# PacificBiosciences/ccs

Measured on AMD Instinct MI355X. Metric: ZMWs/sec (HiFi reads/sec), 10-pass x 10 kb synthetic, higher is better.
Workload: dtype f32

## Files before the change

ccs_amd/csrc/ccsx_api.cpp:

```cpp
#include <hip/hip_runtime.h>

#include <algorithm>
#include <cmath>
#include <cstdio>
#include <cstdlib>
#include <cstring>
#include <initializer_list>
#include <mutex>
#include <string>
#include <vector>

#include "ccsx.h"
#include "ccsx_internal.h"
#include "ccsx_kernels.h"

#define HIPTRY(expr)                                                                                           \
    do {                                                                                                       \
        hipError_t e_ = (expr);                                                                                \
        if (e_ != hipSuccess) {                                                                                \
            ccsx_set_error(std::string(#expr) + ": " + hipGetErrorString(e_));                                 \
            return -2;                                                                                         \
        }                                                                                                      \
    } while (0)

// ... 124 lines not shown
    int device = 0;
    hipStream_t s_in = nullptr, s_draft = nullptr, s_comp = nullptr, s_out = nullptr;
    hipStream_t s_aux = nullptr;
    hipEvent_t ev_epoch = nullptr, ev_epoch_nx = nullptr;
    float age_ms = 0.0f;
    double epoch_ms = 0.0;
    bool poisoned = false;
    ccsx_model model;
    ccsx_opts opts;
    DevBuf d_model, d_poa, d_align;
    DevBuf d_hd_lf;
    Slot slot[CCSX_SLOTS];
    int last = 0;
    int64_t next_ticket = 0;
    int handles_on_device = 1;
};

static void finish_outputs(const Slot &S, ccsx_results *res, ccsx_drafts *d)
{
    const int n = S.P.n_zmw;
    if (res && res->seq_off) std::memcpy(res->seq_off, S.seq_off.p, (size_t)(n + 1) * 8);
    if (d) {
        std::memcpy(d->seq_off, S.seq_off.p, (size_t)(n + 1) * 8);
        if (d->win_off) for (int z = 0; z <= n; ++z) d->win_off[z] = S.wb_off[z];
        for (int z = 0; z < n; ++z) d->backbone[z] &= 255;
    }
}

static int slot_timings(ccsx_handle h, Slot &S, ccsx_timings *t)
{
// ... 87 lines not shown
    else HIPTRY(hipStreamCreateWithFlags(&h->s_comp, hipStreamNonBlocking));
    if (h->opts.serial_stages) h->s_draft = h->s_comp;
    else if (pe) HIPTRY(hipStreamCreateWithPriority(&h->s_draft, hipStreamNonBlocking, p_draft));
    else HIPTRY(hipStreamCreateWithFlags(&h->s_draft, hipStreamNonBlocking));
    HIPTRY(hipStreamCreateWithFlags(&h->s_out, hipStreamNonBlocking));
    { const char *e = getenv("CCSX_POA_SPLIT"); if (((!h->opts.serial_stages && pe) || (e && !strcmp(e, "2"))) && !(e && !strcmp(e, "0"))) { if (pe) HIPTRY(hipStreamCreateWithPriority(&h->s_aux, hipStreamNonBlocking, p_draft)); else HIPTRY(hipStreamCreateWithFlags(&h->s_aux, hipStreamNonBlocking)); } }
    HIPTRY(hipEventCreate(&h->ev_epoch));
    HIPTRY(hipEventCreate(&h->ev_epoch_nx));
    HIPTRY(hipEventRecord(h->ev_epoch, h->s_draft));
    for (auto &s : h->slot) {
        for (auto &ev : s.ev) HIPTRY(hipEventCreate(&ev));
        for (auto &ev : s.ev_aux) HIPTRY(hipEventCreateWithFlags(&ev, hipEventDisableTiming));
        HIPTRY(hipEventCreateWithFlags(&s.ev_up, hipEventDisableTiming));
        HIPTRY(hipEventCreateWithFlags(&s.ev_done, hipEventDisableTiming));
    }
    if (h->d_model.reserve(sizeof(ccsx_model))) return -2;
    HIPTRY(hipMemcpy(h->d_model.p, &h->model, sizeof(ccsx_model), hipMemcpyHostToDevice));
    return 0;
}

int ccsx_create(int device_ordinal, const ccsx_model *model, const ccsx_opts *opts, ccsx_handle *out)
{
    if (!model || !opts || !out) { ccsx_set_error("ccsx_create: null argument"); return -1; }
    int n = 0;
    hipError_t e = hipGetDeviceCount(&n);
    if (e != hipSuccess || n <= 0) { ccsx_set_error("ccsx_create: no HIP device available (this library has no CPU fallback)"); return -2; }
    if (device_ordinal < 0 || device_ordinal >= n) { ccsx_set_error("ccsx_create: bad device ordinal"); return -1; }
    HIPTRY(hipSetDevice(device_ordinal));
    hipDeviceProp_t prop;
    HIPTRY(hipGetDeviceProperties(&prop, device_ordinal));
// ... 275 lines not shown
        if ((P.sdust_words = sdust_mask_words(h, S)) < 0) return -1;
    }
    if ((rc = upload_inputs(S, b, kin, st, P)) || (rc = reserve_state(S, (size_t)n, (size_t)R, kin, pile, W.tandem, P))) return rc;
    if ((rc = grow_scratch(h, n, R, T, P))) return rc;
    P.n_zmw = n; P.n_reads = R; P.maxL_max = (int32_t)T.maxL_max; P.vcap_max = (int32_t)T.vcap_max; P.need_max = T.need_max; P.max_reads = T.nr_max;
    P.n_quads = T.n_quads; P.total_wslots = T.total_wslots;
    P.opts = h->opts;
    P.perr_floor = ccsx_perr_floor(h->opts.max_qv);
    P.model = (const ccsx_model *)h->d_model.p;
    if (ccsx_polish_lds(T.nr_max, &P.pw_obs_bytes, &P.pw_gb_floats)) { ccsx_set_error("ccsx_upload: cannot size the polish kernel's LDS"); return -2; }
    S.P = P;
    S.staged = true; S.ran = false; S.tm_ok = false;
    return 0;
}

static int launch(ccsx_handle h, Slot &S)
{
    (void)hipGetLastError();
    KParams &P = S.P;
    if ((size_t)P.poa_slots * P.poa_slot_bytes > h->d_poa.cap) P.poa_slots = (int)slots_that_fit(h->d_poa.cap, P.poa_slot_bytes, 1);
    const size_t words = h->d_align.cap / 4;
    if ((size_t)P.align_slots * P.align_slot_i32 + align16_words(P.align16_regions, P.align16_slots, P.align16_slot_i32) > words) {
        if ((size_t)P.align_slots * P.align_slot_i32 > words / 2) P.align_slots = (int)slots_that_fit(words / 2, P.align_slot_i32, 1);
        const size_t used = (size_t)P.align_slots * P.align_slot_i32, left = words > used ? words - used : 0;
        P.align16_slots = (int)slots_that_fit(left, (size_t)P.align16_regions * P.align16_slot_i32, 1);
    }
    bind_scratch(h, P);
    if (!h->d_poa.p || !h->d_align.p) { ccsx_set_error("kernel launch refused: the POA / alignment scratch is not allocated (an earlier allocation failed)"); return -2; }
    const char *failed = ccsx_launch_all(S.P, {h->s_draft, h->s_comp, h->s_aux, S.ev, h->s_aux ? S.ev_aux : nullptr}, S.mode);
    if (failed) { ccsx_set_error(std::string("kernel launch failed: ") + failed); return -2; }
    S.ran = true;
    return 0;
}

static int check_results(const Slot &S, const ccsx_results *res, bool have_kin)
{
    const int n = S.P.n_zmw;
    if (!res || res->n_zmw != n || res->seq_capacity < S.seq_off[n]) { ccsx_set_error("ccsx_download: result buffers too small"); return -1; }
    if (!have_kin && (res->fi || res->fp || res->ri || res->rp)) {
        ccsx_set_error("ccsx_download: kinetics buffers given but the handle was created without opts.hifi_kinetics");
        return -1;
    }
    return 0;
}
// ... 859 lines not shown
```

ccs_amd/csrc/ccsx_host.cpp:

```cpp
#include "ccsx.h"
#include "ccsx_internal.h"

int ccsx_kernel_is_experiment();
const char *ccsx_kernel_build_flags();

#include <atomic>
#include <algorithm>
#include <cmath>
#include <thread>
#include <cstdlib>
#include <cstring>
#include <cctype>
#include <cstdio>
#include <sched.h>
#include <string>
#include <vector>

static thread_local std::string g_last_error;
void ccsx_set_error(const std::string &s) { g_last_error = s; }

extern "C" {

int ccsx_abi_version(void) { return CCSX_ABI_VERSION; }
int ccsx_spec_version(void) { return ccsx_kernel_is_experiment() ? -CCSX_SPEC_VERSION : CCSX_SPEC_VERSION; }
const char *ccsx_build_flags(void) { return ccsx_kernel_build_flags(); }
const char *ccsx_last_error(void) { return g_last_error.c_str(); }
const char *ccsx_runtime_switches(void)
{
    static const char *names[] = {"CCSX_STAGE_PRIO", "CCSX_POA_SPLIT", "CCSX_SERIAL_STAGES", "CCSX_A16_ONE_REGION", "CCSX_ALIGN16_MAX_SLOTS", "CCSX_TB_ASIDE",
                                  "CCSX_POLISH_MAX_BLOCKS", "CCSX_EPOCH_REBASE_MS", "CCSX_TRACE", "CCSX_NUMA", "CCSX_INFLATE_PRIO"};
    static thread_local std::string out;
    out.clear();
    for (const char *n : names)
        if (const char *v = std::getenv(n)) { if (!out.empty()) out += ' '; out += n; out += '='; out += v; }
    return out.c_str();
}

void ccsx_model_default(ccsx_model *m)
{
    std::memset(m, 0, sizeof(*m));
    std::strncpy(m->name, "SYN-1", sizeof(m->name) - 1);
    m->snr_lo = 4.0f;
    m->snr_hi = 20.0f;
    static const float pw_match[3] = {0.30f, 0.30f, 0.40f};
    static const float pw_extra[3] = {0.60f, 0.25f, 0.15f};
// ... 248 lines not shown
```

ccs_amd/csrc/ccsx_kernels.h:

```cpp
#pragma once
#include <hip/hip_runtime.h>
#include <stdint.h>
#include <math.h>

#include "ccsx.h"

#define CCSX_POA_BYTES_PER_VERTEX 238

static inline float ccsx_perr_floor(int max_qv) { return max_qv == 50 ? 1e-5f : (float)pow(10.0, -(double)max_qv / 10.0); }

#define CCSX_TB_WORDS_PER_BLOCK 18
static inline __host__ __device__ int ccsx_tb_blocks(int Ld) { return (Ld + 15) >> 4; }
static inline __host__ __device__ int ccsx_tb_stride(int Ld) { return (ccsx_tb_blocks(Ld) * CCSX_TB_WORDS_PER_BLOCK + 3) & ~3; }

static inline __host__ __device__ int ccsx_top_passes(int top_passes) { return (top_passes <= 0 || top_passes > CCSX_MAX_PASSES) ? CCSX_MAX_PASSES : top_passes; }

struct KParams {
    int32_t n_zmw, n_reads;
    int32_t maxL_max;
    int32_t vcap_max;
    int32_t need_max;
    int32_t max_reads;
    int32_t qv_only;
    ccsx_opts opts;
// ... 133 lines not shown
    CCSX_EV_END = 5,
    CCSX_EV_POLISH_START = 6,
    CCSX_EV_COUNT
};
enum ccsx_order_event {
    CCSX_ORD_POA_FORK = 0,
    CCSX_ORD_FIRST_DP_DONE = 1,
    CCSX_ORD_POA_JOIN = 2,
    CCSX_ORD_ALIGN16_DONE_0 = 3,
    CCSX_ORD_ALIGN16_DONE_1 = 4,
    CCSX_ORD_TB_DONE_0 = 5,
    CCSX_ORD_TB_DONE_1 = 6,
    CCSX_ORD_COUNT
};

struct ccsx_launch_queues {
    hipStream_t draft, polish, aux;
    hipEvent_t *ev, *ev_aux;
};
const char *ccsx_launch_all(const KParams &P, const ccsx_launch_queues &q, int mode);
const char *ccsx_train_launch(const KParams &P, hipStream_t st, long long max_blocks);
int ccsx_kernel_is_experiment();
const char *ccsx_kernel_build_flags();
int ccsx_polish_lds(int max_reads, int *obs_bytes, int *gb_floats);
```

ccs_amd/csrc/ccsx_kernels.hip:

```cpp
#include <hip/hip_runtime.h>
#include <stdint.h>
#include <cstdio>
#include <cstdlib>

#include "ccsx.h"
#include "ccsx_kernels.h"
#include "wave_ops.h"

#define LANDED(x) asm volatile("" : "+v"(x))

#if (defined(CCSX_EXP_NO_FILL) || defined(CCSX_EXP_NO_SCORE) || defined(CCSX_EXP_ONE_ROUND) || defined(CCSX_EXP_ALL_VALID) || defined(CCSX_EXP_CHEAP_VALIDITY) || \
     defined(CCSX_EXP_NO_ROWS) || defined(CCSX_EXP_NO_SCORE_LOG) || defined(CCSX_EXP_SKIP_ROUND2_SCORE) || defined(CCSX_EXP_NO_QV_EXP) || defined(CCSX_EXP_REPEAT) || defined(CCSX_EXP_NO_BANDMASK) || \
     defined(CCSX_EXP_HOT_PROLOGUE) || defined(CCSX_EXIT_AFTER_PROLOGUE)) && !defined(CCSX_EXPERIMENT)
#error "CCSX_EXP_* / CCSX_EXIT_AFTER_PROLOGUE switches produce wrong results: build them with -DCCSX_EXPERIMENT (never ship such a library)"
#endif
#define CCSX_STR2(x) #x
#define CCSX_STR(x) CCSX_STR2(x)
int ccsx_kernel_is_experiment()
{
#ifdef CCSX_EXPERIMENT
    return 1;
#else
    return 0;
#endif
// ... 380 lines not shown
                    const int c = 8 + offs[k];
                    bool bad = false;
#pragma unroll
                    for (int p = 1; p <= 4; ++p) bad |= ((e[p - 1] >> (c - p)) & ((1u << p) - 1u)) == ((1u << p) - 1u);
                    if (!bad) nb = cur + CCSX_WIN_CORE + offs[k];
                }
            }
            ++nw;
            if (lane == 0) b[nw] = nb;
            cur = nb;
        }
    }
    return nw;
}

__global__ __launch_bounds__(64) void k_poa_init(KParams P, int z0, int pass, int b0)
{
    const int bx = (int)blockIdx.x + b0;
    const int lane = threadIdx.x;
    uint32_t *sread = dyn_lds;
    PoaSlot g = poa_slot(P, bx);
    if (z0 + bx >= P.n_zmw) return;
    const int z = rfl(P.zmw_perm[z0 + bx]);
    if (lane < ST_WORDS) g.st[lane] = 0;
    __threadfence_block();
    const int r0 = rfl(P.read_off[z]);
    int nreads = rfl(P.read_off[z + 1]) - r0;
    {
        const int top = ccsx_top_passes(P.opts.top_passes);
        if (nreads > top) nreads = top;
    }
    const int nall = nreads;
    {
        int nf = 0;
// ... 56 lines not shown
    else {
        for (int i = lane; i < I; i += LANES) {
            const int b = read_base_packed(sread, i);
            g.crec0[i] = make_int4(b | ((i > 0 ? 1 : 0) << 8) | (1 << CREC_NREADS_SHIFT), i - 1, -1, -1);
            g.needK[i] = 0;
        }
        n = I;
    }
    __threadfence_block();
    if (lane == 0) {
        g.st[ST_N] = n; g.st[ST_NADDED] = 1; g.st[ST_OK] = ok; g.st[ST_PAR] = 0; g.st[ST_KEND] = -1; g.st[ST_BS] = NEGV;
        g.st[ST_NPOA] = npoa; g.st[ST_BB] = bb; g.st[ST_NREADS] = nreads; g.st[ST_REV0] = rev0; g.st[ST_LIVE] = 1;
    }
}

__global__ __launch_bounds__(64) void k_draft_in(KParams P)
{
    const int lane = threadIdx.x, z = blockIdx.x;
    if (z >= P.n_zmw) return;
    const int r0 = rfl(P.read_off[z]);
    int nreads = rfl(P.read_off[z + 1]) - r0;
    {
        const int top = ccsx_top_passes(P.opts.top_passes);
        if (nreads > top) nreads = top;
    }
    const int nall = nreads;
    {
        int nf = 0;
        for (int b0 = 0; b0 < nall; b0 += LANES) nf += __popcll(__ballot(b0 + lane < nall && !(P.flags[r0 + (b0 + lane < nall ? b0 + lane : 0)] & 2)));
        nreads = rfl(nf);
// ... 11 lines not shown
    for (int q = lane; q < Ld; q += LANES) draft[q] = draft[q] & 3;
    __threadfence_block();
    if (stat < 0) nw = poa_windows(P, z, Ld, lane);
    for (int q = lane; q < nall; q += LANES) { P.avalid[r0 + q] = 0; P.ascore[r0 + q] = NEGV; }
    if (lane == 0) {
        P.nreads_used[z] = nall; P.nfull[z] = nreads; P.zref[z] = bb;
        P.draft_len[z] = (stat == CCSX_TOO_FEW_PASSES) ? 0 : Ld; P.nwin[z] = (stat < 0) ? nw : 0; P.zstat[z] = (stat < 0) ? CCSX_SUCCESS : stat;
    }
}

__device__ __forceinline__ void load_read_chunk_m1(uint32_t *sread, const uint8_t *bases, int L, int rev, int c0, int l16)
{
    for (int w = l16; w <= CH16 / 16 + 1; w += 16) sread[w] = pack16_bases<8>(bases, L, c0 - 1 + (w << 4), rev != 0, rev != 0);
}

__global__ __launch_bounds__(64) void k_poa_dp(KParams P, int z0, int pass, int rr, int b0)
{
    const int bx = (int)blockIdx.x + b0;
    __shared__ __attribute__((aligned(16))) int32_t sRing[4][PRING + 1][PGS];
    __shared__ __attribute__((aligned(16))) int4 sKin[4][PRING + 1];
    __shared__ __attribute__((aligned(16))) int4 sCrec[4][16];
    __shared__ uint32_t sRead[4][CH16 / 16 + 2];
    const int lane = threadIdx.x, gq = lane >> 4, l = lane & 15;
    const int zi = z0 + 4 * bx + gq;
    const bool have = zi < P.n_zmw && 4 * bx + gq < P.poa_slots;
    const PoaSlot G = poa_slot(P, have ? 4 * bx + gq : 4 * bx);
    int32_t *st = G.st;
    int32_t *Mcol = G.M;
    int4 *kinfo = G.kinfo;
    const int par_ = have ? st[ST_PAR] : 0;
    const int4 *crec = par_ ? G.crec1 : G.crec0;
    const int32_t *pxw = (const int32_t *)(par_ ? G.px1 : G.px0);
    const uint8_t *needK = G.needK;
    uint8_t *mvK = G.mvK;
    bool live = have && st[ST_LIVE] && st[ST_OK] && rr < st[ST_NPOA];
    if (!__any(live)) return;
    const int z = have ? P.zmw_perm[zi] : 0;
    const int r0 = P.read_off[z];
// ... 188 lines not shown
            if (__builtin_expect((rec.x & CREC_NEED) != 0, 0)) {
                *(int2 *)Mp = make_int2(b0, b1);
                if (l == 0) *kip = make_int4(lo, cm, br, p0);
            }
        }
    }
#undef M_NE0
#undef M_SLT
#undef M_SGT
#undef M_UGT
#undef LDS_I32
    __threadfence_block();
    if (live && l == 0) { st[ST_KEND] = kend; st[ST_BS] = bs; }
}

__global__ __launch_bounds__(64) __attribute__((amdgpu_waves_per_eu(8, 8))) void k_poa_thread(KParams P, int z0, int pass, int rr, int b0)
{
    const int bx = (int)blockIdx.x + b0;
    __shared__ __attribute__((aligned(16))) uint8_t sMv[TB_BLOCK * POA_MV_BYTES];
    const int lane = threadIdx.x;
    uint32_t *sread = dyn_lds;
    PoaSlot g = poa_slot(P, bx);
    if (z0 + bx >= P.n_zmw) return;
    if (!g.st[ST_LIVE] || !g.st[ST_OK] || rr >= g.st[ST_NPOA]) return;
    TPH_T0();
    const int z = rfl(P.zmw_perm[z0 + bx]);
    const int r0 = rfl(P.read_off[z]);
    const int bb = rfl(g.st[ST_BB]), nreads = rfl(g.st[ST_NREADS]), npoa = rfl(g.st[ST_NPOA]);
    const int r = r0 + (bb + rr < nreads ? bb + rr : bb + rr - nreads);
    const uint8_t *rb = P.bases + P.base_off[r];
    const int I = rfl((int)(P.base_off[r + 1] - P.base_off[r]));
    const int kend = rfl(g.st[ST_KEND]), bsc = rfl(g.st[ST_BS]);
    if (kend < 0 || bsc < I) return;
    const int rev = rfl(((P.flags[r] & 1) != g.st[ST_REV0]) ? 1 : 0);
    const int vcap = rfl(P.vcap[z]);
// ... 216 lines not shown
                        rec.x += 1 << 8;
                        if (P - Pp > PRING) { g.needK[Pp] = 1; if (np == 0) rec.x |= CREC_FAR0; }
                    }
                }
            }
            crec_nx[P] = rec;
            if (((rec.x >> 8) & 15) > 3 || pxdirty) px_nx[P] = pxr;
        }
    }
    __threadfence_block();
    if (lane == 0) { g.st[ST_N] = n; g.st[ST_NADDED] += 1; g.st[ST_PAR] ^= 1; }
    (void)npoa;
    TPH(13);
}

__global__ __launch_bounds__(64) __attribute__((amdgpu_waves_per_eu(8, 8))) void k_poa_finish(KParams P, int z0, int pass, int b0)
{
    const int bx = (int)blockIdx.x + b0;
    const int lane = threadIdx.x;
    PoaSlot g = poa_slot(P, bx);
    if (z0 + bx >= P.n_zmw) return;
    if (!g.st[ST_LIVE]) return;
    const int z = rfl(P.zmw_perm[z0 + bx]);
    const int ok = rfl(g.st[ST_OK]), n = rfl(g.st[ST_N]), nadded = rfl(g.st[ST_NADDED]);
    const int4 *crec = g.st[ST_PAR] ? g.crec1 : g.crec0;
    const int32_t *pxw = (const int32_t *)(g.st[ST_PAR] ? g.px1 : g.px0);
    int Ld = 0, nw = 0, stat = -1;
    if (ok && n > 0) {
        int kbest = -1, sb = NEGV, best_prev = 0;
        for (int kb = 0; kb < n; kb += LANES) {
            const int kkL = kb + lane;
            int4 cL = make_int4(0, -1, -1, -1);
            if (kkL < n) cL = crec[kkL];
            const int nblk = (n - kb) < LANES ? (n - kb) : LANES;
// ... 77 lines not shown
        __threadfence_block();
        if (len <= P.dcap[z]) {
            uint8_t *draft = P.draft + P.seq_off[z];
            for (int q = lane; q < len; q += LANES) draft[q] = tmp[len - 1 - q];
            Ld = len;
        }
        __threadfence_block();
    }
    if (Ld <= 0) stat = CCSX_DRAFT_FAILURE;
    else if (Ld < P.opts.min_length) stat = CCSX_TOO_SHORT;
    else if (Ld > P.opts.max_length) stat = CCSX_TOO_LONG;
    else {
        nw = poa_windows(P, z, Ld, lane);
    }
    if (lane == 0) { P.draft_len[z] = Ld; P.nwin[z] = (stat < 0) ? nw : 0; P.zstat[z] = (stat < 0) ? CCSX_SUCCESS : stat; }
}

__device__ __forceinline__ int need_col(const int32_t *wb, int nw, int Ld, int k)
{
    return k == 0 ? 0 : (k == 2 * nw - 1 ? Ld : wb[(k + 1) >> 1] + ((k & 1) ? -CCSX_WIN_OVERHANG : CCSX_WIN_OVERHANG));
}
struct AlignEnd { int M, O, lo; unsigned K; };
template <int REV>
__device__ __forceinline__ AlignEnd align_pass(const KParams &P, const uint32_t *sread, int I, const uint8_t *d, int Ld, const int32_t *wb, int nw,
                                               int32_t *Osave, int lane)
{
    const int nneed = 2 * nw;
    int32_t *lo_need = Osave + (size_t)P.need_max * 128;
    int32_t *cm_need = lo_need + P.need_max + 64, *br_need = cm_need + P.need_max, *eb_need = br_need + P.need_max;
    int2 *OMsave = (int2 *)Osave;
// ... 86 lines not shown
#define AVALID_TB 2
__device__ __forceinline__ int tb_blocks(int Ld) { return ccsx_tb_blocks(Ld); }
__device__ __forceinline__ int tb_stride(int Ld) { return ccsx_tb_stride(Ld); }
__device__ __forceinline__ unsigned shift_in(unsigned acc, unsigned long long m)
{
    unsigned r; unsigned long long co;
    asm("v_addc_co_u32_e64 %0, %1, %2, %2, %3" : "=v"(r), "=s"(co) : "v"(acc), "s"(m));
    return r;
}
__device__ __forceinline__ int sel_i32(unsigned long long m, int a, int b)
{
    int r;
    asm("v_cndmask_b32_e64 %0, %1, %2, %3" : "=v"(r) : "v"(b), "v"(a), "s"(m));
    return r;
}
__global__ __launch_bounds__(64) void k_align16(KParams P, int qbase, int pass, int region)
{
    const int lane = threadIdx.x, h = lane >> 4, l = lane & 15, rowb = lane & 48;
    uint32_t *sread = dyn_lds;
    uint32_t *Osave = (uint32_t *)(P.align_scratch + ((size_t)region * P.align16_slots + blockIdx.x) * P.align16_slot_i32);
    if (qbase + (int)blockIdx.x >= P.n_quads) return;
    const int qd = rfl(P.quads[qbase + blockIdx.x]);
    const int rfirst = qd >> 2, nq = (qd & 3) + 1;
    const int z = rfl(P.read_zmw[rfirst]);
    const int r0 = rfl(P.read_off[z]);
    const int zr = rfl(P.zref[z]);
    if (pass && !(zr & ZREF_PASSBIT(pass))) return;
    const bool live = h < nq;
    const int r = rfirst + (live ? h : 0);
    if (live && l == 0) { P.avalid[r] = 0; P.ascore[r] = NEGV; }
    if (P.zstat[z] != CCSX_SUCCESS) return;
    const int nused = rfl(P.nreads_used[z]);
    if (rfirst - r0 >= nused) return;
    const bool use = live && (r - r0 < nused);
    if (P.opts.disable_heuristics || (P.tflag && (rfl(P.tflag[z]) & 2))) {
        if (l == 0 && use) { const int idx = atomicAdd(&P.align_retry[0], 1); P.align_retry[16 + idx] = r; }
        return;
// ... 121 lines not shown
    const int sc = (inr && scv > -(1 << 22)) ? scv : NEGV;
    const int valid = (sc > NEGV / 2 && sc >= Ld && !satf) ? 1 : 0;
    if (l == 0 && use) {
        P.ascore[r] = sc;
        if (valid) {
            Osave[4 * (size_t)tbs + h] = (uint32_t)lo;
            P.avalid[r] = AVALID_TB;
        } else {
            P.avalid[r] = 0;
            const int idx = atomicAdd(&P.align_retry[0], 1);
            P.align_retry[16 + idx] = r;
        }
    }
}

#define TBE 2
#define TB_LSTRIDE (TBE * 16 + 2 * TBE + 1)
__global__ __launch_bounds__(64) void k_align16_tb(KParams P, int qbase, int nslots, int region)
{
    __shared__ uint32_t sS[64 * TB_LSTRIDE];
    __shared__ unsigned long long sOff[64];
    __shared__ int sCnt[64];
    const int lane = threadIdx.x;
    const int t = (int)blockIdx.x * 64 + lane;
    const int s = t >> 2, h = t & 3;
    bool act = s < nslots;
    int r = 0;
    if (act) {
        const int qd = P.quads[qbase + s];
        const int rfirst = qd >> 2, nq = (qd & 3) + 1;
        act = h < nq;
        r = rfirst + (act ? h : 0);
        act = act && P.avalid[r] == AVALID_TB;
    }
    if (!__any(act)) return;
    const int z = act ? P.read_zmw[r] : 0;
    const int Ld = act ? P.draft_len[z] : 0, nw = act ? P.nwin[z] : 1;
    const int I = act ? (int)(P.base_off[r + 1] - P.base_off[r]) : 0;
    const int tbs = tb_stride(Ld), nb = tb_blocks(Ld);
// ... 77 lines not shown
                eH = j;
                atedge = true;
            }
        }
        bhi = b0;
        __syncthreads();
    }
    if (act) {
        const int len = eH < 32 ? eH : 32;
        unsigned m1 = len > 0 ? __brev(mk) >> (32 - len) : 0u;
        if (i > 0) m1 |= 1u;
        *(uint4 *)ent = make_uint4(0u, e0, e1, e2r);
        *(uint4 *)dm = make_uint4(0u, m1 & 0x7fffffffu, d0, d1);
        P.avalid[r] = 1;
    }
}

__global__ __launch_bounds__(64) void k_align(KParams P, int pass)
{
    const int lane = threadIdx.x;
    uint32_t *sread = dyn_lds;
    int32_t *Osave = P.retry_scratch + (size_t)blockIdx.x * P.align_slot_i32;
    const int nretry = rfl(P.align_retry[0]);
    for (int it = blockIdx.x; it < nretry; it += gridDim.x) {
    const int r = rfl(P.align_retry[16 + it]);
    const int z = rfl(P.read_zmw[r]);
    const int r0 = rfl(P.read_off[z]);
    const int zr = rfl(P.zref[z]);
    __syncthreads();
    const int Ld = rfl(P.draft_len[z]), nw = rfl(P.nwin[z]);
// ... 2338 lines not shown
            gap = max(gap, max(run + sSeg[t][0], sSeg[t][2]));
            run = sSeg[t][1];
        }
        gap = max(gap, run);
        const ccsx_adapter_opts &o = P.adapt;
        const int first = n_hits ? sV[1] : -1, last = sV[2];
        int v = 0;
        if (n_hits >= o.min_copies && gap <= o.max_insert) v |= CCSX_ADAPTER_CONCAT;
        if (n_hits >= 1 && (first <= o.end_slack || last >= L - o.end_slack)) v |= CCSX_ADAPTER_NEAR_END;
        put_planes(out, n, 1, v, n_hits, n_listed, sV[4], gap, first, last, sV[3]);
    }
}

namespace {

struct LaunchSwitches {
    bool trace;
    bool tb_aside;
    long long max_blocks;
    LaunchSwitches()
    {
        const char *aside = getenv("CCSX_TB_ASIDE"), *blocks = getenv("CCSX_POLISH_MAX_BLOCKS");
        const long long v = blocks ? atoll(blocks) : 0;
        trace = getenv("CCSX_TRACE") != nullptr;
        tb_aside = !(aside && aside[0] == '0');
        max_blocks = v > 8 ? (v & ~7ll) : (1ll << 24) - 256;
    }
};

template <typename T, typename F> inline void for_each_piece(T total, T max, F fn)
{
    for (T first = 0; first < total; first += max) fn(first, (total - first) < max ? (total - first) : max);
}

struct Schedule {
    const KParams &P;
    const ccsx_launch_queues &q;
    const LaunchSwitches &sw;
    const hipStream_t st;
    const bool second_stream;
    const bool caller_drafts;
    const size_t lds_read;
    const char *failed = nullptr;

    Schedule(const KParams &P_, const ccsx_launch_queues &q_, int mode, const LaunchSwitches &sw_)
        : P(P_), q(q_), sw(sw_), st(q_.draft), second_stream(q_.aux && q_.ev_aux), caller_drafts(mode == CCSX_RUN_POLISH || mode == CCSX_RUN_HD || mode == CCSX_RUN_TRAIN),
          lds_read((((size_t)P_.maxL_max + 15) / 16) * 4 + 64 + 4 * (CCSX_MAX_PASSES + 1)) {}

    void check(hipError_t e, const char *name) { if (e != hipSuccess && !failed) failed = name; }
    template <typename... KA, typename... A>
    void launch(const char *name, void (*kernel)(KA...), dim3 grid, dim3 block, size_t lds, hipStream_t s, const A &... args)
    {
        hipLaunchKernelGGL(kernel, grid, block, lds, s, args...);
        check(hipGetLastError(), name);
    }
    void record(hipEvent_t e, hipStream_t s) { check(hipEventRecord(e, s), "hipEventRecord"); }
    void wait(hipStream_t s, hipEvent_t e) { check(hipStreamWaitEvent(s, e, 0), "hipStreamWaitEvent"); }
    void memset(void *p, size_t bytes, hipStream_t s) { check(hipMemsetAsync(p, 0, bytes, s), "hipMemsetAsync"); }
    void trace_sync(hipStream_t s, const char *what) const
    {
        if (!sw.trace) return;
        hipError_t e = hipStreamSynchronize(s);
// ... 21 lines not shown
        memset(P.ticket_poa, 256, st);
        memset(P.avalid, (size_t)(P.n_reads > 0 ? P.n_reads : 1), st);
        if (P.tflag) { memset(P.tflag, (size_t)P.n_zmw * 4, st); memset(P.tlen, (size_t)P.n_zmw * 4, st); }
        launch("k_setup", k_setup, dim3((P.n_zmw * CCSX_NCTX + 255) / 256), dim3(256), 0, st, P);
        trace_sync(st, "k_setup");
        stage_event(CCSX_EV_TABLES_DONE, st);
    }

    void poa_round(int pass)
    {
        int cov = pass ? 2 * P.opts.max_poa_cov : P.opts.max_poa_cov;
        if (cov > PW_MAXREADS_SPEC) cov = PW_MAXREADS_SPEC;
        if (cov > P.max_reads) cov = P.max_reads;
        for_each_piece(P.n_zmw, P.poa_slots, [&](int z0, int nb) {
            auto poa_range = [&](hipStream_t s, int g0, int ng, hipEvent_t after_first_dp, hipEvent_t before_first_dp) {
                launch("k_poa_init", k_poa_init, dim3(ng), dim3(64), lds_read, s, P, z0, pass, g0);
                if (before_first_dp) wait(s, before_first_dp);
                for (int rr = 1; rr < cov && pass < 2; ++rr) {
                    launch("k_poa_dp", k_poa_dp, dim3((ng + 3) / 4), dim3(64), 0, s, P, z0, pass, rr, g0 / 4);
                    if (rr == 1 && after_first_dp) record(after_first_dp, s);
                    launch("k_poa_thread", k_poa_thread, dim3(ng), dim3(64), lds_read, s, P, z0, pass, rr, g0);
                }
                if (pass < 2) launch("k_poa_finish", k_poa_finish, dim3(ng), dim3(64), 0, s, P, z0, pass, g0);
            };
            if (second_stream && pass == 0 && cov > 1 && nb >= 4096) {
                const int ha = ((nb / 2) + 3) & ~3;
                record(q.ev_aux[CCSX_ORD_POA_FORK], st);
                wait(q.aux, q.ev_aux[CCSX_ORD_POA_FORK]);
                poa_range(st, 0, ha, q.ev_aux[CCSX_ORD_FIRST_DP_DONE], nullptr);
                poa_range(q.aux, ha, nb - ha, nullptr, q.ev_aux[CCSX_ORD_FIRST_DP_DONE]);
                record(q.ev_aux[CCSX_ORD_POA_JOIN], q.aux);
                wait(st, q.ev_aux[CCSX_ORD_POA_JOIN]);
            } else poa_range(st, 0, nb, nullptr, nullptr);
        });
    }

    void align_cascade(int pass)
    {
        memset(P.align_retry, 64, st);
        const size_t lds16 = 4 * (CH16 / 16 + 3) * sizeof(uint32_t);
        const bool aside = sw.tb_aside && second_stream && pass == 0 && P.n_quads >= 4096;
        int launches = 0;
        for_each_piece(P.n_quads, P.align16_slots, [&](int qb, int nb) {
            const int c = launches++;
            const int region = P.align16_regions > 1 ? (c & 1) : 0;
            if (aside && c >= 2) wait(st, tb_done(c));
            if (aside && c >= 1 && P.align16_regions <= 1) wait(st, tb_done(c - 1));
            launch("k_align16", k_align16, dim3(nb), dim3(64), lds16, st, P, qb, pass, region);
            if (aside) { record(align16_done(c), st); wait(q.aux, align16_done(c)); }
            launch("k_align16_tb", k_align16_tb, dim3((4 * nb + 63) / 64), dim3(64), 0, aside ? q.aux : st, P, qb, nb, region);
            if (aside) record(tb_done(c), q.aux);
        });
        launch("k_align", k_align, dim3(P.align_slots < 1 ? 1 : (P.align_slots > 4096 ? 4096 : P.align_slots)), dim3(64), lds_read, st, P, pass);
        trace_sync(st, "k_align");
        if (P.align_slots >= 2)
            launch("k_rescue", k_rescue, dim3(P.align_slots / 2 > 2048 ? 2048 : P.align_slots / 2), dim3(64), lds_read, st, P, pass);
        if (aside) for (int c = launches > 2 ? launches - 2 : 0; c < launches; ++c) wait(st, tb_done(c));
    }

    void draft_stage()
    {
        if (caller_drafts) launch("k_draft_in", k_draft_in, dim3(P.n_zmw), dim3(64), 0, st, P);
        const int passes = (P.opts.no_fallback_draft || caller_drafts) ? 1 : 3;
        for (int pass = 0; pass < passes; ++pass) {
            if (!caller_drafts) poa_round(pass);
// ... 61 lines not shown
            const char *const name = kin ? (pile ? "k_kinetics_pile" : "k_kinetics") : "k_pileup";
            for_each_piece(P.total_wslots, sw.max_blocks, [&](long long s0, long long nb) {
                launch(name, kfn, dim3(((unsigned)nb + 7u) & ~7u), dim3(256), 0, sp, P, (int)s0);
            });
            trace_sync(sp, "k_kinetics");
        }
        stage_event(CCSX_EV_POLISH_DONE, sp);
        launch("k_stitch", k_stitch, dim3(P.n_zmw), dim3(64), 0, sp, P);
        if (P.out_pile) launch("k_pile_stitch", k_pile_stitch, dim3(P.n_zmw), dim3(64), 0, sp, P);
        stage_event(CCSX_EV_END, sp);
    }
};

}

const char *ccsx_launch_all(const KParams &P, const ccsx_launch_queues &q, int mode)
{
    static const LaunchSwitches switches;
    Schedule s(P, q, mode, switches);
    s.tables();
    s.draft_stage();
    if (mode == CCSX_RUN_DRAFT) {
        s.close_timing(CCSX_EV_DRAFT_STAGE_DONE, CCSX_EV_END);
        return s.failed;
    }
    s.window_map();
    if (mode == CCSX_RUN_FUSED) {
        s.draft_screens();
        if (P.hd_zi) {
            s.hd_finder(false);
            if (P.hd_split) s.window_map();
            s.trace_sync(q.draft, "k_hd");
        }
    }
// ... 16 lines not shown
```

Measured before the change: 38500.

## Add persistent grid-stride draft kernels with a CU budget capped while polish runs

Turns the POA and align16 draft kernels into grid-stride persistent loops, reading params from the kernarg pointer, so the grid can be smaller than the item count. Adds a per-device budget built from kernel register and LDS usage that limits draft waves per CU when another slot's polish is still running. The goal is to leave CU resources to the concurrent polish stage. The default share is 0, so the cap is off unless env vars are set and only the loop wrapper and kernarg changes run, which may add a little overhead.

```diff
diff --git a/ccs_amd/csrc/ccsx_api.cpp b/ccs_amd/csrc/ccsx_api.cpp
--- a/ccs_amd/csrc/ccsx_api.cpp
+++ b/ccs_amd/csrc/ccsx_api.cpp
@@ -162,6 +162,7 @@
     int last = 0;
     int64_t next_ticket = 0;
     int handles_on_device = 1;
+    ccsx_draft_budget budget{};
 };
 
 static void finish_outputs(const Slot &S, ccsx_results *res, ccsx_drafts *d)
@@ -279,6 +280,9 @@
         HIPTRY(hipEventCreateWithFlags(&s.ev_up, hipEventDisableTiming));
         HIPTRY(hipEventCreateWithFlags(&s.ev_done, hipEventDisableTiming));
     }
+    int cus = 0;
+    HIPTRY(hipDeviceGetAttribute(&cus, hipDeviceAttributeMultiprocessorCount, h->device));
+    if (const char *k = ccsx_draft_budget_init(&h->budget, cus)) { ccsx_set_error(std::string("hipFuncGetAttributes(") + k + ") failed"); return -2; }
     if (h->d_model.reserve(sizeof(ccsx_model))) return -2;
     HIPTRY(hipMemcpy(h->d_model.p, &h->model, sizeof(ccsx_model), hipMemcpyHostToDevice));
     return 0;
@@ -584,8 +588,19 @@
     return 0;
 }
 
+static bool polish_in_flight(ccsx_handle h, const Slot &S)
+{
+    if (S.mode != CCSX_RUN_FUSED || h->s_draft == h->s_comp) return false;
+    bool busy = false;
+    for (const Slot &O : h->slot)
+        if (&O != &S && O.inflight && O.ran && (O.mode == CCSX_RUN_FUSED || O.mode == CCSX_RUN_POLISH) && hipEventQuery(O.ev[CCSX_EV_POLISH_DONE]) == hipErrorNotReady) busy = true;
+    (void)hipGetLastError();
+    return busy;
+}
+
 static int launch(ccsx_handle h, Slot &S)
 {
+    const bool capped = polish_in_flight(h, S);
     (void)hipGetLastError();
     KParams &P = S.P;
     if ((size_t)P.poa_slots * P.poa_slot_bytes > h->d_poa.cap) P.poa_slots = (int)slots_that_fit(h->d_poa.cap, P.poa_slot_bytes, 1);
@@ -597,7 +612,7 @@
     }
     bind_scratch(h, P);
     if (!h->d_poa.p || !h->d_align.p) { ccsx_set_error("kernel launch refused: the POA / alignment scratch is not allocated (an earlier allocation failed)"); return -2; }
-    const char *failed = ccsx_launch_all(S.P, {h->s_draft, h->s_comp, h->s_aux, S.ev, h->s_aux ? S.ev_aux : nullptr}, S.mode);
+    const char *failed = ccsx_launch_all(S.P, {h->s_draft, h->s_comp, h->s_aux, S.ev, h->s_aux ? S.ev_aux : nullptr, &h->budget, capped}, S.mode);
     if (failed) { ccsx_set_error(std::string("kernel launch failed: ") + failed); return -2; }
     S.ran = true;
     return 0;
diff --git a/ccs_amd/csrc/ccsx_host.cpp b/ccs_amd/csrc/ccsx_host.cpp
--- a/ccs_amd/csrc/ccsx_host.cpp
+++ b/ccs_amd/csrc/ccsx_host.cpp
@@ -28,7 +28,7 @@
 const char *ccsx_runtime_switches(void)
 {
     static const char *names[] = {"CCSX_STAGE_PRIO", "CCSX_POA_SPLIT", "CCSX_SERIAL_STAGES", "CCSX_A16_ONE_REGION", "CCSX_ALIGN16_MAX_SLOTS", "CCSX_TB_ASIDE",
-                                  "CCSX_POLISH_MAX_BLOCKS", "CCSX_EPOCH_REBASE_MS", "CCSX_TRACE", "CCSX_NUMA", "CCSX_INFLATE_PRIO"};
+                                  "CCSX_POLISH_MAX_BLOCKS", "CCSX_DRAFT_SHARE", "CCSX_DRAFT_SPLIT", "CCSX_DRAFT_MAX_WAVES", "CCSX_EPOCH_REBASE_MS", "CCSX_TRACE", "CCSX_NUMA", "CCSX_INFLATE_PRIO"};
     static thread_local std::string out;
     out.clear();
     for (const char *n : names)
diff --git a/ccs_amd/csrc/ccsx_kernels.h b/ccs_amd/csrc/ccsx_kernels.h
--- a/ccs_amd/csrc/ccsx_kernels.h
+++ b/ccs_amd/csrc/ccsx_kernels.h
@@ -171,9 +171,24 @@
     CCSX_ORD_COUNT
 };
 
+enum ccsx_draft_kernel { CCSX_DK_POA_INIT = 0, CCSX_DK_POA_DP, CCSX_DK_POA_THREAD, CCSX_DK_POA_FINISH, CCSX_DK_ALIGN16, CCSX_DK_ALIGN16_TB, CCSX_DK_COUNT };
+#define CCSX_POLISH_WG_VGPRS 128
+#define CCSX_POLISH_WG_LDS   (40 * 1024)
+struct ccsx_draft_budget {
+    int share;
+    int split;
+    int max_waves;
+    int cus;
+    int simd_waves[CCSX_DK_COUNT];
+    int lds_static[CCSX_DK_COUNT];
+};
+const char *ccsx_draft_budget_init(ccsx_draft_budget *b, int cus);
+
 struct ccsx_launch_queues {
     hipStream_t draft, polish, aux;
     hipEvent_t *ev, *ev_aux;
+    const ccsx_draft_budget *budget;
+    bool capped;
 };
 const char *ccsx_launch_all(const KParams &P, const ccsx_launch_queues &q, int mode);
 const char *ccsx_train_launch(const KParams &P, hipStream_t st, long long max_blocks);
diff --git a/ccs_amd/csrc/ccsx_kernels.hip b/ccs_amd/csrc/ccsx_kernels.hip
--- a/ccs_amd/csrc/ccsx_kernels.hip
+++ b/ccs_amd/csrc/ccsx_kernels.hip
@@ -418,10 +418,26 @@
     return nw;
 }
 
-__global__ __launch_bounds__(64) void k_poa_init(KParams P, int z0, int pass, int b0)
-{
-    const int bx = (int)blockIdx.x + b0;
-    const int lane = threadIdx.x;
+__device__ __forceinline__ int item_lane()
+{
+    int l = (int)threadIdx.x;
+    asm volatile("" : "+v"(l));
+    __builtin_assume(l >= 0 && l < 64);
+    return l;
+}
+typedef const __attribute__((address_space(4))) KParams *KParamsArg;
+__device__ __forceinline__ const KParams &item_params()
+{
+    KParamsArg p = (KParamsArg)__builtin_amdgcn_kernarg_segment_ptr();
+    asm volatile("" : "+s"(p));
+    return *(const KParams *)p;
+}
+#define FOR_EACH_ITEM(n_items) for (int item = (int)blockIdx.x; item < (n_items); item += (int)gridDim.x, __syncthreads())
+
+__device__ __forceinline__ void poa_init_item(const KParams &P, int z0, int pass, int b0, int item)
+{
+    const int bx = item + b0;
+    const int lane = item_lane();
     uint32_t *sread = dyn_lds;
     PoaSlot g = poa_slot(P, bx);
     if (z0 + bx >= P.n_zmw) return;
@@ -508,6 +524,11 @@
     }
 }
 
+__global__ __launch_bounds__(64) void k_poa_init(KParams P, int z0, int pass, int b0, int n_items)
+{
+    FOR_EACH_ITEM(n_items) poa_init_item(item_params(), z0, pass, b0, item);
+}
+
 __global__ __launch_bounds__(64) void k_draft_in(KParams P)
 {
     const int lane = threadIdx.x, z = blockIdx.x;
@@ -549,14 +570,14 @@
     for (int w = l16; w <= CH16 / 16 + 1; w += 16) sread[w] = pack16_bases<8>(bases, L, c0 - 1 + (w << 4), rev != 0, rev != 0);
 }
 
-__global__ __launch_bounds__(64) void k_poa_dp(KParams P, int z0, int pass, int rr, int b0)
-{
-    const int bx = (int)blockIdx.x + b0;
+__device__ __forceinline__ void poa_dp_item(const KParams &P, int z0, int pass, int rr, int b0, int item)
+{
+    const int bx = item + b0;
     __shared__ __attribute__((aligned(16))) int32_t sRing[4][PRING + 1][PGS];
     __shared__ __attribute__((aligned(16))) int4 sKin[4][PRING + 1];
     __shared__ __attribute__((aligned(16))) int4 sCrec[4][16];
     __shared__ uint32_t sRead[4][CH16 / 16 + 2];
-    const int lane = threadIdx.x, gq = lane >> 4, l = lane & 15;
+    const int lane = item_lane(), gq = lane >> 4, l = lane & 15;
     const int zi = z0 + 4 * bx + gq;
     const bool have = zi < P.n_zmw && 4 * bx + gq < P.poa_slots;
     const PoaSlot G = poa_slot(P, have ? 4 * bx + gq : 4 * bx);
@@ -775,11 +796,16 @@
     if (live && l == 0) { st[ST_KEND] = kend; st[ST_BS] = bs; }
 }
 
-__global__ __launch_bounds__(64) __attribute__((amdgpu_waves_per_eu(8, 8))) void k_poa_thread(KParams P, int z0, int pass, int rr, int b0)
-{
-    const int bx = (int)blockIdx.x + b0;
+__global__ __launch_bounds__(64) void k_poa_dp(KParams P, int z0, int pass, int rr, int b0, int n_items)
+{
+    FOR_EACH_ITEM(n_items) poa_dp_item(item_params(), z0, pass, rr, b0, item);
+}
+
+__device__ __forceinline__ void poa_thread_item(const KParams &P, int z0, int pass, int rr, int b0, int item)
+{
+    const int bx = item + b0;
     __shared__ __attribute__((aligned(16))) uint8_t sMv[TB_BLOCK * POA_MV_BYTES];
-    const int lane = threadIdx.x;
+    const int lane = item_lane();
     uint32_t *sread = dyn_lds;
     PoaSlot g = poa_slot(P, bx);
     if (z0 + bx >= P.n_zmw) return;
@@ -1026,10 +1052,15 @@
     TPH(13);
 }
 
-__global__ __launch_bounds__(64) __attribute__((amdgpu_waves_per_eu(8, 8))) void k_poa_finish(KParams P, int z0, int pass, int b0)
-{
-    const int bx = (int)blockIdx.x + b0;
-    const int lane = threadIdx.x;
+__global__ __launch_bounds__(64) __attribute__((amdgpu_waves_per_eu(8, 8))) void k_poa_thread(KParams P, int z0, int pass, int rr, int b0, int n_items)
+{
+    FOR_EACH_ITEM(n_items) poa_thread_item(item_params(), z0, pass, rr, b0, item);
+}
+
+__device__ __forceinline__ void poa_finish_item(const KParams &P, int z0, int pass, int b0, int item)
+{
+    const int bx = item + b0;
+    const int lane = item_lane();
     PoaSlot g = poa_slot(P, bx);
     if (z0 + bx >= P.n_zmw) return;
     if (!g.st[ST_LIVE]) return;
@@ -1137,6 +1168,11 @@
         nw = poa_windows(P, z, Ld, lane);
     }
     if (lane == 0) { P.draft_len[z] = Ld; P.nwin[z] = (stat < 0) ? nw : 0; P.zstat[z] = (stat < 0) ? CCSX_SUCCESS : stat; }
+}
+
+__global__ __launch_bounds__(64) __attribute__((amdgpu_waves_per_eu(8, 8))) void k_poa_finish(KParams P, int z0, int pass, int b0, int n_items)
+{
+    FOR_EACH_ITEM(n_items) poa_finish_item(item_params(), z0, pass, b0, item);
 }
 
 __device__ __forceinline__ int need_col(const int32_t *wb, int nw, int Ld, int k)
@@ -1253,13 +1289,13 @@
     asm("v_cndmask_b32_e64 %0, %1, %2, %3" : "=v"(r) : "v"(b), "v"(a), "s"(m));
     return r;
 }
-__global__ __launch_bounds__(64) void k_align16(KParams P, int qbase, int pass, int region)
-{
-    const int lane = threadIdx.x, h = lane >> 4, l = lane & 15, rowb = lane & 48;
+__device__ __forceinline__ void align16_item(const KParams &P, int qbase, int pass, int region, int item)
+{
+    const int lane = item_lane(), h = lane >> 4, l = lane & 15, rowb = lane & 48;
     uint32_t *sread = dyn_lds;
-    uint32_t *Osave = (uint32_t *)(P.align_scratch + ((size_t)region * P.align16_slots + blockIdx.x) * P.align16_slot_i32);
-    if (qbase + (int)blockIdx.x >= P.n_quads) return;
-    const int qd = rfl(P.quads[qbase + blockIdx.x]);
+    uint32_t *Osave = (uint32_t *)(P.align_scratch + ((size_t)region * P.align16_slots + item) * P.align16_slot_i32);
+    if (qbase + item >= P.n_quads) return;
+    const int qd = rfl(P.quads[qbase + item]);
     const int rfirst = qd >> 2, nq = (qd & 3) + 1;
     const int z = rfl(P.read_zmw[rfirst]);
     const int r0 = rfl(P.read_off[z]);
@@ -1411,15 +1447,20 @@
     }
 }
 
+__global__ __launch_bounds__(64) void k_align16(KParams P, int qbase, int pass, int region, int n_items)
+{
+    FOR_EACH_ITEM(n_items) align16_item(item_params(), qbase, pass, region, item);
+}
+
 #define TBE 2
 #define TB_LSTRIDE (TBE * 16 + 2 * TBE + 1)
-__global__ __launch_bounds__(64) void k_align16_tb(KParams P, int qbase, int nslots, int region)
+__device__ __forceinline__ void align16_tb_item(const KParams &P, int qbase, int nslots, int region, int item)
 {
     __shared__ uint32_t sS[64 * TB_LSTRIDE];
     __shared__ unsigned long long sOff[64];
     __shared__ int sCnt[64];
-    const int lane = threadIdx.x;
-    const int t = (int)blockIdx.x * 64 + lane;
+    const int lane = item_lane();
+    const int t = item * 64 + lane;
     const int s = t >> 2, h = t & 3;
     bool act = s < nslots;
     int r = 0;
@@ -1527,6 +1568,11 @@
         *(uint4 *)dm = make_uint4(0u, m1 & 0x7fffffffu, d0, d1);
         P.avalid[r] = 1;
     }
+}
+
+__global__ __launch_bounds__(64) void k_align16_tb(KParams P, int qbase, int nslots, int region, int n_items)
+{
+    FOR_EACH_ITEM(n_items) align16_tb_item(item_params(), qbase, nslots, region, item);
 }
 
 __global__ __launch_bounds__(64) void k_align(KParams P, int pass)
@@ -3895,19 +3941,31 @@
 
 namespace {
 
+#define CCSX_DRAFT_SHARE_DEFAULT 0
+#define CCSX_DRAFT_SPLIT_DEFAULT 1
+
 struct LaunchSwitches {
     bool trace;
     bool tb_aside;
     long long max_blocks;
+    int draft_share;
+    int draft_split;
+    int draft_max_waves;
     LaunchSwitches()
     {
         const char *aside = getenv("CCSX_TB_ASIDE"), *blocks = getenv("CCSX_POLISH_MAX_BLOCKS");
+        const char *share = getenv("CCSX_DRAFT_SHARE"), *split = getenv("CCSX_DRAFT_SPLIT"), *waves = getenv("CCSX_DRAFT_MAX_WAVES");
         const long long v = blocks ? atoll(blocks) : 0;
+        draft_share = (share && share[0] >= '0' && share[0] <= '3' && !share[1]) ? share[0] - '0' : CCSX_DRAFT_SHARE_DEFAULT;
+        draft_split = (split && (split[0] == '0' || split[0] == '1') && !split[1]) ? split[0] - '0' : CCSX_DRAFT_SPLIT_DEFAULT;
+        draft_max_waves = waves && atoi(waves) > 0 ? atoi(waves) : 0;
         trace = getenv("CCSX_TRACE") != nullptr;
         tb_aside = !(aside && aside[0] == '0');
         max_blocks = v > 8 ? (v & ~7ll) : (1ll << 24) - 256;
     }
 };
+
+const LaunchSwitches &launch_switches() { static const LaunchSwitches s; return s; }
 
 template <typename T, typename F> inline void for_each_piece(T total, T max, F fn)
 {
@@ -3922,11 +3980,30 @@
     const bool second_stream;
     const bool caller_drafts;
     const size_t lds_read;
+    const bool share_applies;
+    const bool use_second_stream;
     const char *failed = nullptr;
 
     Schedule(const KParams &P_, const ccsx_launch_queues &q_, int mode, const LaunchSwitches &sw_)
         : P(P_), q(q_), sw(sw_), st(q_.draft), second_stream(q_.aux && q_.ev_aux), caller_drafts(mode == CCSX_RUN_POLISH || mode == CCSX_RUN_HD || mode == CCSX_RUN_TRAIN),
-          lds_read((((size_t)P_.maxL_max + 15) / 16) * 4 + 64 + 4 * (CCSX_MAX_PASSES + 1)) {}
+          lds_read((((size_t)P_.maxL_max + 15) / 16) * 4 + 64 + 4 * (CCSX_MAX_PASSES + 1)),
+          share_applies(q_.budget && q_.capped && q_.budget->share > 0 && q_.budget->max_waves <= 0),
+          use_second_stream(second_stream && !(share_applies && !q_.budget->split)) {}
+
+    unsigned draft_grid(ccsx_draft_kernel k, int items, size_t lds_dyn, bool has_company) const
+    {
+        if (items < 1) items = 1;
+        const ccsx_draft_budget *b = q.budget;
+        if (b && b->max_waves > 0) return (unsigned)(items < b->max_waves ? items : b->max_waves);
+        if (!share_applies) return (unsigned)items;
+        long long per_cu = 4ll * b->simd_waves[k];
+        const long long lds = (long long)b->lds_static[k] + (long long)lds_dyn;
+        if (lds > 0 && (long long)b->share * CCSX_POLISH_WG_LDS / lds < per_cu) per_cu = (long long)b->share * CCSX_POLISH_WG_LDS / lds;
+        if (has_company) per_cu /= 2;
+        if (per_cu < 4) per_cu = 4;
+        const long long waves = per_cu * (b->cus > 0 ? b->cus : 1);
+        return (unsigned)(items < waves ? items : waves);
+    }
 
     void check(hipError_t e, const char *name) { if (e != hipSuccess && !failed) failed = name; }
     template <typename... KA, typename... A>
@@ -3978,16 +4055,18 @@
         if (cov > P.max_reads) cov = P.max_reads;
         for_each_piece(P.n_zmw, P.poa_slots, [&](int z0, int nb) {
             auto poa_range = [&](hipStream_t s, int g0, int ng, hipEvent_t after_first_dp, hipEvent_t before_first_dp) {
-                launch("k_poa_init", k_poa_init, dim3(ng), dim3(64), lds_read, s, P, z0, pass, g0);
+                const bool halves = after_first_dp || before_first_dp;
+                launch("k_poa_init", k_poa_init, dim3(draft_grid(CCSX_DK_POA_INIT, ng, lds_read, halves)), dim3(64), lds_read, s, P, z0, pass, g0, ng);
                 if (before_first_dp) wait(s, before_first_dp);
                 for (int rr = 1; rr < cov && pass < 2; ++rr) {
-                    launch("k_poa_dp", k_poa_dp, dim3((ng + 3) / 4), dim3(64), 0, s, P, z0, pass, rr, g0 / 4);
+                    launch("k_poa_dp", k_poa_dp, dim3(draft_grid(CCSX_DK_POA_DP, (ng + 3) / 4, 0, halves)), dim3(64), 0, s, P, z0, pass, rr, g0 / 4, (ng + 3) / 4);
                     if (rr == 1 && after_first_dp) record(after_first_dp, s);
-                    launch("k_poa_thread", k_poa_thread, dim3(ng), dim3(64), lds_read, s, P, z0, pass, rr, g0);
+                    launch("k_poa_thread", k_poa_thread, dim3(draft_grid(CCSX_DK_POA_THREAD, ng, lds_read, halves)), dim3(64), lds_read, s, P, z0, pass, rr, g0, ng);
                 }
-                if (pass < 2) launch("k_poa_finish", k_poa_finish, dim3(ng), dim3(64), 0, s, P, z0, pass, g0);
+                if (pass < 2)
+                    launch("k_poa_finish", k_poa_finish, dim3(draft_grid(CCSX_DK_POA_FINISH, ng, 0, halves)), dim3(64), 0, s, P, z0, pass, g0, ng);
             };
-            if (second_stream && pass == 0 && cov > 1 && nb >= 4096) {
+            if (use_second_stream && pass == 0 && cov > 1 && nb >= 4096) {
                 const int ha = ((nb / 2) + 3) & ~3;
                 record(q.ev_aux[CCSX_ORD_POA_FORK], st);
                 wait(q.aux, q.ev_aux[CCSX_ORD_POA_FORK]);
@@ -4003,16 +4082,16 @@
     {
         memset(P.align_retry, 64, st);
         const size_t lds16 = 4 * (CH16 / 16 + 3) * sizeof(uint32_t);
-        const bool aside = sw.tb_aside && second_stream && pass == 0 && P.n_quads >= 4096;
+        const bool aside = sw.tb_aside && use_second_stream && pass == 0 && P.n_quads >= 4096;
         int launches = 0;
         for_each_piece(P.n_quads, P.align16_slots, [&](int qb, int nb) {
             const int c = launches++;
             const int region = P.align16_regions > 1 ? (c & 1) : 0;
             if (aside && c >= 2) wait(st, tb_done(c));
             if (aside && c >= 1 && P.align16_regions <= 1) wait(st, tb_done(c - 1));
-            launch("k_align16", k_align16, dim3(nb), dim3(64), lds16, st, P, qb, pass, region);
+            launch("k_align16", k_align16, dim3(draft_grid(CCSX_DK_ALIGN16, nb, lds16, aside && c >= 1)), dim3(64), lds16, st, P, qb, pass, region, nb);
             if (aside) { record(align16_done(c), st); wait(q.aux, align16_done(c)); }
-            launch("k_align16_tb", k_align16_tb, dim3((4 * nb + 63) / 64), dim3(64), 0, aside ? q.aux : st, P, qb, nb, region);
+            launch("k_align16_tb", k_align16_tb, dim3(draft_grid(CCSX_DK_ALIGN16_TB, (4 * nb + 63) / 64, 0, aside)), dim3(64), 0, aside ? q.aux : st, P, qb, nb, region, (4 * nb + 63) / 64);
             if (aside) record(tb_done(c), q.aux);
         });
         launch("k_align", k_align, dim3(P.align_slots < 1 ? 1 : (P.align_slots > 4096 ? 4096 : P.align_slots)), dim3(64), lds_read, st, P, pass);
@@ -4104,10 +4183,27 @@
 
 }
 
+const char *ccsx_draft_budget_init(ccsx_draft_budget *b, int cus)
+{
+    const LaunchSwitches &switches = launch_switches();
+    const struct { const void *kernel; const char *name; } kernels[CCSX_DK_COUNT] = {
+        {(const void *)k_poa_init, "k_poa_init"}, {(const void *)k_poa_dp, "k_poa_dp"}, {(const void *)k_poa_thread, "k_poa_thread"},
+        {(const void *)k_poa_finish, "k_poa_finish"}, {(const void *)k_align16, "k_align16"}, {(const void *)k_align16_tb, "k_align16_tb"}};
+    b->share = switches.draft_share; b->split = switches.draft_split; b->max_waves = switches.draft_max_waves; b->cus = cus;
+    for (int k = 0; k < CCSX_DK_COUNT; ++k) {
+        hipFuncAttributes a;
+        if (hipFuncGetAttributes(&a, kernels[k].kernel) != hipSuccess) { (void)hipGetLastError(); return kernels[k].name; }
+        const int regs = a.numRegs > 0 ? (a.numRegs + 7) & ~7 : CCSX_POLISH_WG_VGPRS;
+        const int w = b->share * CCSX_POLISH_WG_VGPRS / regs;
+        b->simd_waves[k] = w > 8 ? 8 : w;
+        b->lds_static[k] = (int)a.sharedSizeBytes;
+    }
+    return nullptr;
+}
+
 const char *ccsx_launch_all(const KParams &P, const ccsx_launch_queues &q, int mode)
 {
-    static const LaunchSwitches switches;
-    Schedule s(P, q, mode, switches);
+    Schedule s(P, q, mode, launch_switches());
     s.tables();
     s.draft_stage();
     if (mode == CCSX_RUN_DRAFT) {
```

New measurement: 38510, median of 4. About the same (+0.0%).
